# wendongbi/Bridged-GNN

Measured on AMD Instinct MI355X. Metric: aggregated_edges_per_sec_ktgnn_fwd, higher is better.
Workload: dtype f32; 1 GPU; C4 synthetic bridged graph (local) N=1000000 E'=20991058, 2-layer KT-GNN eval fwd F=128 hidden=128 C=2; parallelism=single, execution=eager launches

## Files before the change

bridged_gnn_amd/_lib.py:

```python
import ctypes as C
import os

import torch

_HERE = os.path.dirname(os.path.abspath(__file__))
SO_PATH = os.path.join(_HERE, "csrc", "libbgnn_hip.so")
_lib = None

_P, _I64, _I32, _F32, _SZ, _INT = C.c_void_p, C.c_int64, C.c_int32, C.c_float, C.c_size_t, C.c_int

SIGNATURES = {
    "bgnn_version": (_INT, []),
    "bgnn_source_hash": (C.c_char_p, []),
    "bgnn_error_string": (C.c_char_p, [_INT]),
    "bgnn_csr_workspace_bytes": (_SZ, [_I64, _I64]),
    "bgnn_build_dst_csr": (_INT, [_P, _I64, _I64, _INT, _P, _P, _P, _P, _P, _SZ, _P]),
    "bgnn_domain_sums_f64": (_INT, [_P, _I64, _I32, _I64, _P, _P, _P]),
    "bgnn_domain_sums_workspace_bytes": (_SZ, [_I32]),
    "bgnn_domain_sums_ws_f64": (_INT, [_P, _I64, _I32, _I64, _P, _P, _P, _SZ, _P]),
    "bgnn_domain_delta_f32": (_INT, [_P, _I32, _P, _P]),
    "bgnn_adaptedconv_transform_f32": (_INT, [_P, _I64, _I32, _I64, _P, _P, _I32, _I32, _P, _P, _P, _P,
                                               _P, _P, _P, _P, _I64, _I64, _P, _P]),
    "bgnn_adaptedconv_transform_sums_f32": (_INT, [_P, _I64, _I32, _I64, _P, _P, _I32, _I32, _P, _P, _P, _P,
                                                    _P, _P, _P, _P, _I64, _I64, _I64, _I64, _P, _P]),
# ... 4 lines not shown
    "bgnn_classifier_stage_f32": (_INT, [_P, _I64, _I32, _I64, _P, _P, _I32, _I32, _P, _P, _P, _P, _P, _P, _P, _P, _I64, _I64,
                                          _P, _P, _I32, _INT, _P, _P, _P, _P, _P, _P]),
    "bgnn_linear_narrow_transform_f32": (_INT, [_P, _I64, _I32, _I64, _P, _P, _I32, _INT, _P, _P, _P, _P, _P, _P]),
    "bgnn_narrow_transform_finish_f32": (_INT, [_P, _I64, _P, _P, _I32, _P, _P, _P, _P, _P, _P, _I64, _P, _P]),
    "bgnn_gram_workspace_bytes": (C.c_size_t, [_I32, _I32]),
    "bgnn_gram_f32": (_INT, [_P, _I64, _I32, _P, _I64, _I32, _I64, _P, _P, C.c_size_t, _P]),
    "bgnn_transform_bwd_prep_workspace_bytes": (C.c_size_t, [_I64, _I32]),
    "bgnn_transform_bwd_prep_f32": (_INT, [_P, _I64, _I64, _I32, _P, _P, _I64, _I32, _P, _P, _P, _P, _P, _P, _I32, _I64, _P, _I64, _P, _P, C.c_size_t, _P]),
    "bgnn_bn_acc_doubles": (_I64, [_I32]),
    "bgnn_bn_relu_dropout_f32": (_INT, [_P, _I64, _I32, _I64, _P, _P, _F32, _INT, _F32, C.c_uint64, _P, _F32, _P, _P, _P, _I64, _P, _P]),
    "bgnn_bn_relu_dropout_bwd_f32": (_INT, [_P, _P, _I64, _I32, _I64, _I64, _P, _P, _P, _F32, _INT, _F32, C.c_uint64, _P, _P, _I64, _P, _P]),
    "bgnn_bn_colstats_f32": (_INT, [_P, _I64, _I32, _I64, _P, _P]),
    "bgnn_bn_apply_rows_f32": (_INT, [_P, _I64, _I32, _I64, _P, _I64, _P, _P, _F32, _INT, _F32, C.c_uint64, _P, _P, _I64, _F32, _P, _P, _P, _I64, _P]),
    "bgnn_bn_bwd_reduce_rows_f32": (_INT, [_P, _P, _I64, _I32, _I64, _I64, _P, _I64, _P, _P, _F32, _INT, _F32, C.c_uint64, _P, _P, _I64, _P, _P]),
    "bgnn_bn_bwd_apply_rows_f32": (_INT, [_P, _P, _I64, _I32, _I64, _I64, _P, _P, _I64, _P, _P, _F32, _INT, _F32, C.c_uint64, _P, _P, _I64, _P, _I64, _P]),
    "bgnn_transform_bwd_consts_f32": (_INT, [_P, _P, _P, _P, _P, _I32, _I32, _P, _P, _P, _P]),
    "bgnn_transform_bwd_finish_f32": (_INT, [_P, _P, _P, _P, _P, _P, _P, _I32, _I32, _I32, _P, _P, _P, _P, _P, _P, _P, _I64, _P]),
    "bgnn_rowdot_f32": (_INT, [_P, _I64, _I64, _I32, _P, _I64, _I32, _P, _P]),
    "bgnn_linear_f32": (_INT, [_P, _I64, _I32, _I64, _P, _P, _I32, _INT, _P, _P, _P, _I64, _P]),
    "bgnn_adaptedconv_aggregate_f32": (_INT, [_P, _P, _I64, _P, _P, _P, _P, _P, _I64, _I64, _I32, _F32,
                                               _P, _I64, _P, _P, _P, _INT, _P, _INT, _I64, _I32, _P, _P, _P]),
    "bgnn_adaptedconv_aggregate_bounded_f32": (_INT, [_P, _P, _I64, _P, _P, _P, _P, _P, _I64, _I64, _I32, _F32,
                                                       _P, _I64, _P, _P, _P, _INT, _P, _INT, _I64, _I32, _P, _P, _I64, _I32, _P]),
    "bgnn_aggregate_hub_workspace_bytes": (C.c_size_t, [_I64, _I32, _I64]),
    "bgnn_adaptedconv_aggregate_hub_f32": (_INT, [_P, _P, _I64, _P, _P, _P, _P, _P, _I64, _I32, _F32, _P, _I64, _P, _P, _INT, _P, _I32, _P,
                                                   _P, _I32, _P, _I64, _P, _P, _P, _I64, _P, _P, C.c_size_t, _P]),
    "bgnn_adaptedconv_aggregate_bwd_f32": (_INT, [_P, _P, _I64, _P, _P, _P, _P, _P, _I64, _I64, _I32, _F32,
                                                   _P, _I64, _P, _P, _I64, _P, _P, _P, _P, _P]),
    "bgnn_aggregate_bwd_pull_workspace_bytes": (C.c_size_t, [_I64, _I64, _I64, _I32, _I64, _I64]),
    "bgnn_adaptedconv_aggregate_bwd_pull_f32": (_INT, [_P, _P, _I64, _P, _P, _P, _P, _P, _P, _P, _P, _I64, _I64, _I32, _F32,
                                                        _P, _I64, _P, _P, _I64, _P, _P, _P, _P, _I32,
                                                        _P, _I64, _P, _P, _P, _I64, _P, _I64, _P, _P, _P, _I64, _P, C.c_size_t, _P]),
    "bgnn_aggregate_heads_bwd_workspace_bytes": (C.c_size_t, [_I64, _I64, _I32, _I64, _I64]),
    "bgnn_adaptedconv_aggregate_heads_bwd_f32": (_INT, [_P, _P, _P, _P, _P, _P, _P, _P, _P, _I64, _I64, _I32, _I32, _F32,
                                                         _P, _P, _P, _INT, _P, _P, _P, _P, _I32,
                                                         _P, _I64, _P, _P, _P, _I64, _P, _I64, _P, _P, _P, _I64, _P, C.c_size_t, _P]),
    "bgnn_adaptedconv_aggregate_heads_wide_f32": (_INT, [_P, _P, _I64, _P, _P, _P, _P, _P, _I64, _I32, _I32, _F32, _P, _P, _P]),
    "bgnn_aggregate_heads_wide_bwd_workspace_bytes": (C.c_size_t, [_I64, _I32, _I64]),
    "bgnn_adaptedconv_aggregate_heads_wide_bwd_f32": (_INT, [_P, _P, _I64, _P, _P, _P, _P, _P, _P, _P, _I64, _I32, _I32, _F32,
                                                              _P, _P, _P, _P, _P, _P, _P, _P, C.c_size_t, _P]),
    "bgnn_l2_normalize_rows_f32": (_INT, [_P, _I64, _I32, _F32, _P, _P]),
    "bgnn_topk_workspace_bytes": (_SZ, [_I64, _I64, _I32]),
    "bgnn_cosine_topk_f32": (_INT, [_P, _P, _I64, _I64, _I32, _I32, _INT, _P, _P, _P, _P, _SZ, _P]),
    "bgnn_mlp_pair_topk_f32": (_INT, [_P, _P, _P, _P, _P, _F32, _I64, _I64, _I32, _I32, _INT, _P, _P, _P,
                                       _P, _SZ, _P]),
    "bgnn_topk_edges_i64": (_INT, [_P, _I64, _I32, _I64, _I64, _P, _P]),
# ... 175 lines not shown
```

bridged_gnn_amd/csrc/bgnn_aggregate.hip:

```cpp
#include <cstdlib>
#include "bgnn_common.h"

namespace {

struct AggParams {
  const float* h_t2s;
  const float* h_s2t;
  int64_t ldh;
  const float* a_t2s;
  const float* a_s2t;
  const int32_t* rowptr;
  const int32_t* col;
  const uint8_t* mask;
  int64_t row_begin;
  int64_t row_end;
  int32_t D;
  float slope;
  float* out;
  int64_t ldo;
  float* alpha;
  const float* ep_scale;
  const float* ep_shift;
  int ep_relu;
  unsigned int* tile_queue;
  double* colsum;
  int32_t heads;
  float* state_ms;
  int mode;
  int64_t park_begin;
  int tq_chunk;
  int tq_interleave;
  int xcd_segments;
  const int32_t* vrow_node;
  const int32_t* vrow_bounds;
  int64_t n_vrows;
  float* vout; float* vms;
  int32_t hub_threshold;
  const char* tbl_base;
  uint32_t tbl_bytes, off_t2s, off_s2t;
  int32_t gather_hint;
  uint32_t dead_off;
};

__device__ __forceinline__ float leaky(float v, float slope) { return v > 0.f ? v : v * slope; }

template <int LF, int EP, int U>
__global__ __launch_bounds__(256) void agg_kernel(AggParams p) {
  constexpr int GL = LF * EP;
  constexpr int GPW = 64 / GL;
  constexpr int RPB = 4 * GPW;
  const int lane = threadIdx.x & 63;
  const int wave = threadIdx.x >> 6;
  const int g = lane / GL;
  const int lg = lane % GL;
  const int sub = lg / LF;
  const int f0 = (lg % LF) * 4;
  const bool fvalid = f0 < p.D;

  const int64_t ntiles = ((p.row_end - p.row_begin) * p.heads + RPB - 1) / RPB;
  bgnn::XcdRange tr = bgnn::xcd_pos_range(ntiles);
  __shared__ float red[2][LF * 4 + 1];
  if (p.colsum != nullptr) {
    for (int t = threadIdx.x; t < 2 * (LF * 4 + 1); t += 256) (&red[0][0])[t] = 0.f;
    __syncthreads();
// ... 429 lines not shown
      if (p.colsum != nullptr) {
        if (dom_s) { cs_s.x += o.x; cs_s.y += o.y; cs_s.z += o.z; cs_s.w += o.w; n_s += 1.f; }
        else       { cs_t.x += o.x; cs_t.y += o.y; cs_t.z += o.z; cs_t.w += o.w; n_t += 1.f; }
      }
    }
  }
  if (p.colsum != nullptr) {
    unsafeAtomicAdd(&red[0][f0], cs_s.x); unsafeAtomicAdd(&red[0][f0 + 1], cs_s.y);
    unsafeAtomicAdd(&red[0][f0 + 2], cs_s.z); unsafeAtomicAdd(&red[0][f0 + 3], cs_s.w);
    unsafeAtomicAdd(&red[1][f0], cs_t.x); unsafeAtomicAdd(&red[1][f0 + 1], cs_t.y);
    unsafeAtomicAdd(&red[1][f0 + 2], cs_t.z); unsafeAtomicAdd(&red[1][f0 + 3], cs_t.w);
    if (lg == 0) { unsafeAtomicAdd(&red[0][LF * 4], n_s); unsafeAtomicAdd(&red[1][LF * 4], n_t); }
    __syncthreads();
    for (int t = threadIdx.x; t < 2 * (LF * 4 + 1); t += 256) {
      const int d = t / (LF * 4 + 1), c = t % (LF * 4 + 1);
      const double sum = (double)red[d][c];
      if (c == LF * 4) unsafeAtomicAdd(&p.colsum[2 * p.ldo + d], sum);
      else if (c < p.ldo) unsafeAtomicAdd(&p.colsum[d * p.ldo + c], sum);
    }
  }
}

typedef unsigned int u32x4_t __attribute__((ext_vector_type(4)));

template <int CTRL>
__device__ __forceinline__ uint32_t dpp_movu(uint32_t x) { return (uint32_t)__builtin_amdgcn_update_dpp(0, (int)x, CTRL, 0xF, 0xF, true); }

template <int LF, bool ALPHA>
__global__ __launch_bounds__(256) void agg_wide_fast_kernel(AggParams p) {
  static_assert(LF == 16 || LF == 32 || LF == 64, "wide rows only");
  constexpr int U = 4;
  constexpr int GPW = 64 / LF;
  constexpr int RPB = 4 * GPW;
  const int lane = threadIdx.x & 63;
  const int wave = threadIdx.x >> 6;
  const int g = lane / LF;
  const int lg = lane % LF;
  const int f0 = lg * 4;
  const bool fvalid = f0 < p.D;
  const int f0c = fvalid ? f0 : 0;
  const int k = lane & (U - 1);
  const bool b0 = lane & 1, b1 = lane & 2;

  const int32_t row0 = (int32_t)p.row_begin, row1 = (int32_t)p.row_end;
  const int32_t ntiles = (row1 - row0 + RPB - 1) / RPB;
  __shared__ float red[2][LF * 4 + 1];
  if (p.colsum != nullptr) {
    for (int t = threadIdx.x; t < 2 * (LF * 4 + 1); t += 256) (&red[0][0])[t] = 0.f;
    __syncthreads();
  }
  __shared__ unsigned int dyn_tile;
  const uint32_t nstride = (uint32_t)(p.ldh * 4);
  const uint32_t ostride = (uint32_t)(p.ldo * 4);
  const __amdgpu_buffer_rsrc_t rt = __builtin_amdgcn_make_buffer_rsrc(const_cast<char*>(p.tbl_base), (short)0, (int)p.tbl_bytes, 0x00020000);
  const __amdgpu_buffer_rsrc_t ro = __builtin_amdgcn_make_buffer_rsrc(p.out, (short)0, (int)((uint32_t)row1 * ostride), 0x00020000);
  const f2 sl = {p.slope, p.slope};
  float sc4[4] = {0.f, 0.f, 0.f, 0.f}, sh4[4] = {0.f, 0.f, 0.f, 0.f};
  if (p.ep_scale != nullptr) {
#pragma unroll
    for (int c = 0; c < 4; ++c)
      if (f0 + c < p.D) { sc4[c] = p.ep_scale[f0 + c]; sh4[c] = p.ep_shift[f0 + c]; }
  }
  f2 cs_s01 = {0.f, 0.f}, cs_s23 = cs_s01, cs_t01 = cs_s01, cs_t23 = cs_s01;
  float n_s = 0.f, n_t = 0.f;
  f2 aS01 = {0.f, 0.f}, aS23 = aS01, aT01 = aS01, aT23 = aS01;
  if (fvalid) {
    aS01.x = p.a_t2s[f0]; aS01.y = f0 + 1 < p.D ? p.a_t2s[f0 + 1] : 0.f;
    aS23.x = f0 + 2 < p.D ? p.a_t2s[f0 + 2] : 0.f; aS23.y = f0 + 3 < p.D ? p.a_t2s[f0 + 3] : 0.f;
    aT01.x = p.a_s2t[f0]; aT01.y = f0 + 1 < p.D ? p.a_s2t[f0 + 1] : 0.f;
    aT23.x = f0 + 2 < p.D ? p.a_s2t[f0 + 2] : 0.f; aT23.y = f0 + 3 < p.D ? p.a_s2t[f0 + 3] : 0.f;
  }
  const int32_t TQ_CHUNK = p.tq_chunk;
  const int32_t xcd = blockIdx.x % 8, slot = blockIdx.x / 8;
  const int32_t G = ((int32_t)gridDim.x + 7 - xcd) / 8;
  const int32_t tstride = p.tq_interleave ? G : 1;
  const int32_t NSEG = p.xcd_segments > 1 ? p.xcd_segments : 1;
  const int32_t per_x = (ntiles + 7) / 8, seg_len = (per_x + NSEG - 1) / NSEG;
  const int32_t xbase = xcd * per_x;
  const int32_t xend = NSEG > 1 ? xbase + NSEG * seg_len : min((xcd + 1) * per_x, ntiles);
  int32_t tile = xbase + slot - G;
  int32_t chunk_left = 0;
  for (;;) {
    if (p.tile_queue != nullptr) {
      if (chunk_left == 0) {
        __syncthreads();
        if (threadIdx.x == 0) dyn_tile = atomicAdd(&p.tile_queue[xcd], 1u);
        __syncthreads();
        const uint32_t kq = dyn_tile;
        if (p.tq_interleave) {
          const int32_t sc = (int32_t)kq / G, r = (int32_t)kq - sc * G;
          tile = xbase + sc * (TQ_CHUNK * G) + r;
        } else {
          tile = xbase + (int32_t)kq * TQ_CHUNK;
        }
        chunk_left = TQ_CHUNK;
        if (tile >= xend) break;
      } else {
        tile += tstride;
      }
      --chunk_left;
      if (tile >= xend) { chunk_left = 0; continue; }
    } else {
      tile += G;
      if (tile >= xend) break;
    }
    int32_t gt = tile;
    if (NSEG > 1) {
      const int32_t j = tile - xbase, sg = j / seg_len;
      gt = (sg * 8 + xcd) * seg_len + (j - sg * seg_len);
      if (gt >= ntiles) continue;
    }
    const int32_t i0 = row0 + gt * RPB + wave * GPW + g;
    const bool rvalid = i0 < row1;
    const int32_t ic = rvalid ? i0 : row0;
    const bool dom_s = p.mask[ic] != 0;
    const int32_t beg = rvalid ? p.rowptr[ic] : 0;
    const int32_t end = rvalid ? p.rowptr[ic + 1] : 0;
    const uint32_t lbase = (dom_s ? p.off_t2s : p.off_s2t) + (uint32_t)f0c * 4u;
    const f2 a01 = dom_s ? aS01 : aT01, a23 = dom_s ? aS23 : aT23;
    const float4 hi4 = __builtin_bit_cast(float4, __builtin_amdgcn_raw_buffer_load_b128(rt, lbase + __umul24((uint32_t)ic, nstride), 0, 0));
    f2 h01 = {hi4.x, hi4.y}, h23 = {hi4.z, hi4.w};

    float m = -INFINITY, s = 0.f;
    f2 acc01 = {0.f, 0.f}, acc23 = {0.f, 0.f};
    const int32_t niter = (end - beg + U - 1) / U;
    auto issue = [&](float4 (&v)[U], uint32_t off) {
      v[0] = __builtin_bit_cast(float4, __builtin_amdgcn_raw_buffer_load_b128(rt, lbase + dpp_movu<0x00>(off), 0, 0));
      v[1] = __builtin_bit_cast(float4, __builtin_amdgcn_raw_buffer_load_b128(rt, lbase + dpp_movu<0x55>(off), 0, 0));
      v[2] = __builtin_bit_cast(float4, __builtin_amdgcn_raw_buffer_load_b128(rt, lbase + dpp_movu<0xAA>(off), 0, 0));
      v[3] = __builtin_bit_cast(float4, __builtin_amdgcn_raw_buffer_load_b128(rt, lbase + dpp_movu<0xFF>(off), 0, 0));
      asm volatile("" : "+v"(h01), "+v"(h23) : : "memory");
      __builtin_amdgcn_sched_barrier(0);
    };
// ... 42 lines not shown
#define BGNN_ACC(u, w)                                               \
      {                                                              \
        acc01.x = fmaf(w, v[u].x, acc01.x); acc01.y = fmaf(w, v[u].y, acc01.y); \
        acc23.x = fmaf(w, v[u].z, acc23.x); acc23.y = fmaf(w, v[u].w, acc23.y); \
      }
#ifdef AGGF_X_NOACC
      acc01.x += pe * v[0].x + v[1].y + v[2].z + v[3].w;
#else
      { const float w = quad_bcast<0>(pe); BGNN_ACC(0, w) }
      { const float w = quad_bcast<1>(pe); BGNN_ACC(1, w) }
      { const float w = quad_bcast<2>(pe); BGNN_ACC(2, w) }
      { const float w = quad_bcast<3>(pe); BGNN_ACC(3, w) }
#endif
#undef BGNN_ACC
      m = mn;
    };
    int32_t nw = __builtin_amdgcn_readlane(niter, 0);
    if constexpr (LF <= 32) nw = max(nw, __builtin_amdgcn_readlane(niter, 32));
    if constexpr (LF <= 16) nw = max(nw, max(__builtin_amdgcn_readlane(niter, 16), __builtin_amdgcn_readlane(niter, 48)));
    int32_t e = beg + k;
    bool ok = e < end;
    uint32_t myoff = p.dead_off;
    if (nw > 0) myoff = row_off((uint32_t)p.col[max(min(e, end - 1), 0)], ok);
    for (int32_t it = 0; it < nw; ++it) {
      float4 v[U];
      issue(v, myoff);
      const int32_t e_cur = e;
      e += U;
      const bool ok2 = e < end;
      uint32_t nextid = load_id(e);
      update(v, ok, e_cur);
      ok = ok2;
      take_id(nextid);
      myoff = row_off(nextid, ok);
    }
    s += bgnn::dpp_mov<0xB1>(s);
    s += bgnn::dpp_mov<0x4E>(s);

    const float inv = 1.f / (s + 1e-16f);
    if constexpr (ALPHA) {
      if (lg < U) {
        for (int32_t e2 = beg + lg; e2 < end; e2 += 4 * U) {
          float a[4];
#pragma unroll
          for (int j = 0; j < 4; ++j) a[j] = e2 + j * U < end ? p.alpha[e2 + j * U] : 0.f;
#pragma unroll
          for (int j = 0; j < 4; ++j)
            if (e2 + j * U < end) p.alpha[e2 + j * U] = __expf(a[j] - m) * inv;
        }
      }
    }
    if (rvalid && f0 < p.ldo) {
      float4 o = make_float4(acc01.x * inv, acc01.y * inv, acc23.x * inv, acc23.y * inv);
      if (p.ep_scale != nullptr) {
        o.x = fmaf(o.x, sc4[0], sh4[0]); o.y = fmaf(o.y, sc4[1], sh4[1]);
        o.z = fmaf(o.z, sc4[2], sh4[2]); o.w = fmaf(o.w, sc4[3], sh4[3]);
      }
// ... 231 lines not shown
  return 0;
}

static bool fast_plan(AggParams& p, int64_t table_rows) {
  static const bool on = [] { const char* e = getenv("BGNN_AGG_FAST"); return !(e && atoi(e) == 0); }();
  if (!on || table_rows <= 0) return false;
  if (p.heads != 1 || p.mode != 0 || p.n_vrows != 0 || p.hub_threshold != 0) return false;
  const int64_t lim24 = (int64_t)1 << 24, lim32 = ((int64_t)1 << 32) - 1;
  if (table_rows > lim24 || p.row_end > table_rows || p.ldh * 4 >= lim24 || p.ldo * 4 >= lim24) return false;
  const char* a = reinterpret_cast<const char*>(p.h_t2s);
  const char* b = reinterpret_cast<const char*>(p.h_s2t);
  const char* lo = a < b ? a : b;
  const int64_t span = (int64_t)((a < b ? b : a) - lo) + table_rows * p.ldh * 4;
  if (span > lim32 || p.row_end * p.ldo * 4 > lim32) return false;
  p.tbl_base = lo;
  p.tbl_bytes = (uint32_t)span;
  p.off_t2s = (uint32_t)(a - lo);
  p.off_s2t = (uint32_t)(b - lo);
  const int64_t lane_max = (span - table_rows * p.ldh * 4) + p.ldh * 4, dead = (((int64_t)1 << 32) - 16) - lane_max;
  p.dead_off = dead >= span ? (uint32_t)dead : 0u;
  return true;
}

template <int LF, bool ALPHA>
int launch_wide_fast(const AggParams& p, hipStream_t st) {
  constexpr int RPB = 4 * (64 / LF);
  static const int per_cu_max = [] {
    int per_cu = 0;
    if (hipOccupancyMaxActiveBlocksPerMultiprocessor(&per_cu, agg_wide_fast_kernel<LF, ALPHA>, 256, 0) != hipSuccess || per_cu < 1) return 0;
    if (per_cu > 8) per_cu = 8;
    const char* e = getenv("BGNN_AGG_BLOCKS_PER_CU");
    if (e && atoi(e) > 0 && atoi(e) < per_cu) per_cu = atoi(e);
    return per_cu;
  }();
  static const int n_cu = [] {
    int dev = 0;
    hipDeviceProp_t prop;
    if (hipGetDevice(&dev) != hipSuccess || hipGetDeviceProperties(&prop, dev) != hipSuccess) return 0;
    return prop.multiProcessorCount;
  }();
  static const bool forced = getenv("BGNN_AGG_BLOCKS_PER_CU") != nullptr;
  int per_cu = per_cu_max;
  if (p.gather_hint == 2 && !forced && per_cu > 3) per_cu = 3;
  const int64_t cap = (per_cu_max > 0 && n_cu > 0) ? (int64_t)per_cu * n_cu / 8 * 8 : 2048;
  const int64_t ntiles = (p.row_end - p.row_begin + RPB - 1) / RPB;
  int64_t grid = ntiles < cap ? (ntiles + 7) / 8 * 8 : cap;
  if (grid < 8) grid = 8;
  AggParams q = p;
  q.tq_chunk = tq_chunk_for(ntiles, grid);
  static const int il = [] { const char* e = getenv("BGNN_AGG_INTERLEAVE"); return e ? atoi(e) : 1; }();
  q.tq_interleave = il;
  static const int nseg = [] { const char* e = getenv("BGNN_XCD_SEGMENTS"); return e ? atoi(e) : 8; }();
  q.xcd_segments = nseg;
  hipLaunchKernelGGL((agg_wide_fast_kernel<LF, ALPHA>), dim3((unsigned)grid), dim3(256), 0, st, q);
  BGNN_LAUNCH_CHECK();
  return 0;
}

struct HubMergeParams {
  const int32_t* hub_rows; const int32_t* seg_ptr; int64_t n_hubs;
  const float* part_acc;
  const float* part_ms;
  const uint8_t* mask;
  int32_t D; int64_t ldo; int32_t heads;
  float* out; const float* ep_scale; const float* ep_shift; int ep_relu;
  double* colsum; float* state_ms;
  float* alpha; const int32_t* rowptr;
};

template <int LF>
__global__ __launch_bounds__(256) void hub_merge_wide_kernel(HubMergeParams p) {
  const int lane = threadIdx.x % LF, grp = threadIdx.x / LF;
  constexpr int GPB = 256 / LF;
  const int f0 = lane * 4;
  const bool fvalid = f0 < p.D;
  __shared__ float red[2][LF * 4 + 1];
// ... 137 lines not shown
    if (nv <= 32) return launch_wide<32, 4>(p, st);
    return launch_wide<64, 4>(p, st);
  }
  if (nv <= 16) return launch<16, 1, 8>(p, st);
  if (nv <= 32) return launch<32, 1, 4>(p, st);
  return launch<64, 1, 4>(p, st);
}

static bool hub_capable(int32_t D, int64_t ldh, int64_t ldo, int32_t heads, float slope) {
  if ((heads == 3 || heads == 2) && D <= 4 && ldh == 4 && ldo == 4) return true;
  const int nv = (D + 3) / 4;
  return heads == 1 && nv > 8 && slope >= 0.f && slope <= 1.f && ldh * 4 < (int64_t)1 << 32;
}

}

static int aggregate_impl(const float* h_t2s, const float* h_s2t, int64_t ldh,
                          const float* a_t2s, const float* a_s2t,
                          const int32_t* rowptr, const int32_t* col, const uint8_t* mask,
                          int64_t row_begin, int64_t row_end, int32_t D, float negative_slope,
                          float* out, int64_t ldo, float* alpha_opt,
                          const float* ep_scale_opt, const float* ep_shift_opt, int ep_relu,
                          float* state_ms_opt, int part, int64_t park_begin, int32_t heads,
                          double* colsum_opt, uint32_t* tile_queue_opt, int64_t table_rows, int32_t gather_hint, void* stream) {
  if (colsum_opt && heads != 1) return BGNN_E_SHAPE;
  if (part == 1 && (park_begin < row_begin || park_begin > row_end)) return BGNN_E_SHAPE;
  if (part < 0 || part > 3 || (part != 0 && (!state_ms_opt || alpha_opt))) return BGNN_E_NULL;
  if (part == 3 && !((heads == 3 || heads == 2) && D <= 4 && ldh == 4 && ldo == 4)) return BGNN_E_SHAPE;
  if (heads < 1 || heads > 8 || (heads > 1 && (alpha_opt || ep_scale_opt))) return BGNN_E_SHAPE;
  if (ep_relu < 0 || ep_relu > 2) return BGNN_E_SHAPE;
  if (ep_relu == 2 && !((heads == 3 || heads == 2) && D <= 4 && ldh == 4 && ldo == 4)) return BGNN_E_SHAPE;
  if (!h_t2s || !h_s2t || !a_t2s || !a_s2t || !rowptr || !col || !mask || !out) return BGNN_E_NULL;
  if (row_begin < 0 || row_end < row_begin || D <= 0 || D > 256 || ldh < D || ldo < D) return BGNN_E_SHAPE;
  if ((ldh & 3) || (ldo & 3) || !bgnn_aligned16(h_t2s) || !bgnn_aligned16(h_s2t) || !bgnn_aligned16(out))
    return BGNN_E_ALIGN;
  if ((ep_scale_opt == nullptr) != (ep_shift_opt == nullptr)) return BGNN_E_NULL;
  if (row_end == row_begin) return 0;
  AggParams p{h_t2s, h_s2t, ldh, a_t2s, a_s2t, rowptr, col, mask, row_begin, row_end, D, negative_slope,
              out, ldo, alpha_opt, ep_scale_opt, ep_shift_opt, ep_relu, tile_queue_opt, colsum_opt, heads, state_ms_opt, part,
              park_begin, 4};
  p.gather_hint = gather_hint;
  hipStream_t st = (hipStream_t)stream;
  if (tile_queue_opt) {
    hipError_t e = bgnn_zero_async(tile_queue_opt, 8 * sizeof(uint32_t), st);
    if (e != hipSuccess) return (int)e;
  }
  return dispatch_aggregate(p, st, table_rows);
}

extern "C" int bgnn_adaptedconv_aggregate_f32(const float* h_t2s, const float* h_s2t, int64_t ldh,
                                              const float* a_t2s, const float* a_s2t,
                                              const int32_t* rowptr, const int32_t* col, const uint8_t* mask,
                                              int64_t row_begin, int64_t row_end, int32_t D, float negative_slope,
                                              float* out, int64_t ldo, float* alpha_opt,
                                              const float* ep_scale_opt, const float* ep_shift_opt, int ep_relu,
                                              float* state_ms_opt, int part, int64_t park_begin, int32_t heads,
                                              double* colsum_opt, uint32_t* tile_queue_opt, void* stream) {
  return aggregate_impl(h_t2s, h_s2t, ldh, a_t2s, a_s2t, rowptr, col, mask, row_begin, row_end, D, negative_slope, out, ldo, alpha_opt,
                        ep_scale_opt, ep_shift_opt, ep_relu, state_ms_opt, part, park_begin, heads, colsum_opt, tile_queue_opt, 0, 0, stream);
}

extern "C" int bgnn_adaptedconv_aggregate_bounded_f32(const float* h_t2s, const float* h_s2t, int64_t ldh,
                                                      const float* a_t2s, const float* a_s2t,
                                                      const int32_t* rowptr, const int32_t* col, const uint8_t* mask,
                                                      int64_t row_begin, int64_t row_end, int32_t D, float negative_slope,
                                                      float* out, int64_t ldo, float* alpha_opt,
                                                      const float* ep_scale_opt, const float* ep_shift_opt, int ep_relu,
                                                      float* state_ms_opt, int part, int64_t park_begin, int32_t heads,
                                                      double* colsum_opt, uint32_t* tile_queue_opt, int64_t table_rows, int32_t gather_hint,
                                                      void* stream) {
  if (table_rows < row_end || gather_hint < 0 || gather_hint > 2) return BGNN_E_SHAPE;
  return aggregate_impl(h_t2s, h_s2t, ldh, a_t2s, a_s2t, rowptr, col, mask, row_begin, row_end, D, negative_slope, out, ldo, alpha_opt,
                        ep_scale_opt, ep_shift_opt, ep_relu, state_ms_opt, part, park_begin, heads, colsum_opt, tile_queue_opt, table_rows, gather_hint, stream);
}

extern "C" size_t bgnn_aggregate_hub_workspace_bytes(int64_t n_segments, int32_t heads, int64_t ldo) {
  const size_t nv = (size_t)(n_segments > 0 ? n_segments : 0), h = (size_t)(heads > 0 ? heads : 1);
  return bgnn_align_up(sizeof(float) * nv * h * (size_t)(ldo > 0 ? ldo : 0), 256) + bgnn_align_up(sizeof(float) * 2 * nv * h, 256) + 256;
}

extern "C" int bgnn_adaptedconv_aggregate_hub_f32(const float* h_t2s, const float* h_s2t, int64_t ldh,
                                                  const float* a_t2s, const float* a_s2t,
                                                  const int32_t* rowptr, const int32_t* col, const uint8_t* mask,
                                                  int64_t N, int32_t D, float negative_slope, float* out, int64_t ldo,
                                                  const float* ep_scale_opt, const float* ep_shift_opt, int ep_relu,
                                                  float* state_ms_opt, int32_t heads, double* colsum_opt,
                                                  uint32_t* tile_queue_opt, int32_t hub_threshold, const int32_t* hub_rows,
                                                  int64_t n_hubs, const int32_t* hub_seg_ptr, const int32_t* seg_bounds,
                                                  const int32_t* seg_node, int64_t n_segments, float* alpha_opt,
                                                  void* ws, size_t ws_bytes, void* stream) {
  if (!h_t2s || !h_s2t || !a_t2s || !a_s2t || !rowptr || !col || !mask || !out) return BGNN_E_NULL;
  if (alpha_opt && heads != 1) return BGNN_E_SHAPE;
  if (n_hubs > 0 && (!hub_rows || !hub_seg_ptr || !seg_bounds || !seg_node || !ws)) return BGNN_E_NULL;
  if (N < 0 || D <= 0 || D > 256 || ldh < D || ldo < D || (ldh & 3) || (ldo & 3) || hub_threshold < 2 || n_hubs < 0 || n_segments < n_hubs)
    return BGNN_E_SHAPE;
  if (!hub_capable(D, ldh, ldo, heads, negative_slope)) return BGNN_E_SHAPE;
// ... 84 lines not shown
```

bridged_gnn_amd/ops.py:

```python
import ctypes
import os

import torch

from . import _lib as L

__all__ = ["DstCSR", "build_dst_csr", "domain_delta", "pack_transform_heads", "adaptedconv_transform", "adaptedconv_aggregate", "linear", "linear_supported", "linear_narrow_supported", "linear_narrow_transform", "narrow_transform_finish", "gram", "gram_supported", "rowdot", "transform_bwd_prep", "topk_edges_coalesced",
           "l2_normalize_rows", "cosine_topk", "mlp_pair_topk", "topk_edges", "coalesce", "gather_rows", "pad4",
           "sage_mean_aggregate", "sage_mean_aggregate_bwd", "rows_segment_add", "gcn_aggregate", "gcn_aggregate_bwd", "gat_scores", "gat_aggregate", "gat_aggregate_bwd", "gatv2_aggregate", "gatv2_aggregate_bwd", "wide_heads_supported",
           "adaptedconv_aggregate_heads_wide", "adaptedconv_aggregate_heads_wide_bwd", "pair_csr", "pair_mlp_stats", "pair_mlp_loss",
           "pair_mlp_segsum", "pair_mlp_eval", "pair_mlp_count", "PAIR_MLP_WIDTH", "pair_cos_loss", "pair_cos_segsum", "pair_cos_count",
           "PAIR_COS_WIDTH"]


def pad4(n):
    return (int(n) + 3) // 4 * 4


HUB_THRESHOLD = 128
HUB_SEGMENT = 64


class DstCSR:

# ... 512 lines not shown
    if tile_need is not None:
        if delta is not None or tuple(tail_single) != (0, 0):
            raise ValueError("tile_need needs the sums form of the transform and no tail_single")
        if tile_need.dtype != torch.int32 or tile_need.numel() != (N + 31) // 32:
            raise ValueError("tile_need: one int32 per 32-row tile")
        fn, name, tail = lib.bgnn_adaptedconv_transform_need_f32, "bgnn_adaptedconv_transform_need_f32", (L.ptr(tile_need),)
    if delta is None and H == 1 and (tile_need is not None or tail_single[0] or tail_single[1]):
        c = getattr(tile_need, "_team_plan", None)
        runs = c[1] if (c is not None and c[0] == (N, dev, tile_need._version)) else transform_team_runs(N, dev, tile_need, tail_single)
        if runs:
            flat = (ctypes.c_int64 * (3 * len(runs)))(*[v for r in runs for v in r])
            fn, name = lib.bgnn_adaptedconv_transform_need2_f32, "bgnn_adaptedconv_transform_need2_f32"
            tail = (int(tail_single[0]), int(tail_single[1]), L.ptr(tile_need) if tile_need is not None else None, flat, len(runs))
    rc = fn(L.ptr(x), N, Din, x.stride(0), L.ptr(mask_u8), L.ptr(first), H, D, L.ptr(Wp), L.ptr(bp), L.ptr(gates), L.ptr(gconst),
            L.ptr_rows(out[0][1]), L.ptr_rows(out[0][0]), L.ptr_rows(o1[1]), L.ptr_rows(o1[0]), ldh, row_stride, *tail,
            L.ptr(small), L.stream())
    L.check(rc, name)
    return out


_P2_STATIC = os.environ.get("BGNN_P2_STATIC", "1") != "0"


def _tile_queue(dev):
    return torch.empty(8, dtype=torch.int32, device=dev)


def heads_log_softmax_supported(heads, D):
    return heads in (2, 3) and D <= 4


def _hub_shape_ok(D, ldh, ldo, heads, slope):
    if heads in (2, 3) and D <= 4 and ldh == 4 and ldo == 4:
        return True
    return heads == 1 and D > 32 and 0.0 <= slope <= 1.0


def adaptedconv_aggregate(h_t2s, h_s2t, a_t2s, a_s2t, csr, mask_u8, D, negative_slope=0.1, n_dst=None,
                          want_alpha=False, ep_scale=None, ep_shift=None, ep_relu=False, out=None,
                          row_begin=0, row_end=None, state_ms=None, part=0, heads=1, colsum=None, log_softmax=False,
                          park_begin=None):
    lib = L.lib()
    n_dst = csr.num_nodes if n_dst is None else int(n_dst)
    row_end = n_dst if row_end is None else int(row_end)
    ldh = h_t2s.stride(0) // heads
    ldo = pad4(D)
    dev = h_t2s.device
    if out is None:
# ... 1 lines not shown
    assert h_t2s.stride(0) == h_s2t.stride(0) and h_t2s.stride(0) % heads == 0 and out.stride(0) % heads == 0
    alpha = torch.empty(csr.num_edges, dtype=torch.float32, device=dev) if want_alpha else None
    tq = _tile_queue(dev) if heads == 1 else None
    if row_end <= int(row_begin):
        return (out, alpha) if want_alpha else out
    if ((not want_alpha or heads == 1) and part in (0, 3) and int(row_begin) == 0 and row_end == csr.num_nodes == n_dst and h_t2s.shape[0] == n_dst
            and (ep_scale is None or heads == 1) and _hub_shape_ok(D, ldh, out.stride(0) // heads, heads, negative_slope)
            and os.environ.get("BGNN_HUB_ROWS", "1") != "0"):
        hubs = csr.hub_tables()
        if hubs is not None:
            hub_rows, seg_ptr, seg_bounds, seg_node = hubs
            nseg = int(seg_node.numel())
            wsb = lib.bgnn_aggregate_hub_workspace_bytes(nseg, heads, out.stride(0) // heads)
            ws = torch.empty(wsb, dtype=torch.uint8, device=dev)
            rc = lib.bgnn_adaptedconv_aggregate_hub_f32(
                L.ptr_rows(h_t2s), L.ptr_rows(h_s2t), ldh, L.ptr(a_t2s), L.ptr(a_s2t), L.ptr(csr.rowptr), L.ptr(csr.col),
                L.ptr(mask_u8), n_dst, D, float(negative_slope), L.ptr_rows(out), out.stride(0) // heads,
                L.ptr(ep_scale), L.ptr(ep_shift), 2 if log_softmax else (1 if ep_relu else 0),
                L.ptr(state_ms) if part == 3 else None, int(heads), L.ptr(colsum),
                L.ptr(tq), HUB_THRESHOLD, L.ptr(hub_rows), int(hub_rows.numel()),
                L.ptr(seg_ptr), L.ptr(seg_bounds), L.ptr(seg_node), nseg, L.ptr(alpha), L.ptr(ws), wsb, L.stream())
            L.check(rc, "bgnn_adaptedconv_aggregate_hub_f32")
            return (out, alpha) if want_alpha else out
    rc = lib.bgnn_adaptedconv_aggregate_bounded_f32(
        L.ptr_rows(h_t2s), L.ptr_rows(h_s2t), ldh, L.ptr(a_t2s), L.ptr(a_s2t), L.ptr(csr.rowptr), L.ptr(csr.col),
        L.ptr(mask_u8), int(row_begin), row_end, D, float(negative_slope), L.ptr_rows(out), out.stride(0) // heads, L.ptr(alpha),
        L.ptr(ep_scale), L.ptr(ep_shift), 2 if log_softmax else (1 if ep_relu else 0), L.ptr(state_ms), int(part),
        int(row_begin) if park_begin is None else int(park_begin), int(heads), L.ptr(colsum),
        L.ptr(tq) if not (part == 2 and _P2_STATIC) else None, min(int(h_t2s.shape[0]), int(h_s2t.shape[0])),
        csr.gather_hint() if (heads == 1 and D > 32 and part == 0) else 0, L.stream())
    L.check(rc, "bgnn_adaptedconv_aggregate_bounded_f32")
    return (out, alpha) if want_alpha else out


def _bwd_hub_args(csr, use=True):
    use = use and os.environ.get("BGNN_HUB_ROWS", "1") != "0"
    args, nseg = [HUB_THRESHOLD], []
    for tables in ((csr.hub_tables(), csr.transposed_hub_tables()) if use else (None, None)):
        rows, seg_ptr, bounds, node = tables if tables is not None else (None, None, None, None)
        nseg.append(0 if tables is None else int(node.numel()))
        args += [L.ptr(rows), 0 if tables is None else int(rows.numel()), L.ptr(seg_ptr), L.ptr(bounds), L.ptr(node), nseg[-1]]
    return args, nseg[0], nseg[1]


def adaptedconv_aggregate_bwd(h_t2s, h_s2t, a_t2s, a_s2t, csr, mask_u8, D, out, alpha, grad_out, negative_slope=0.1):
    lib = L.lib()
    dev = h_t2s.device
    da_t2s = torch.zeros(D, dtype=torch.float32, device=dev)
    da_s2t = torch.zeros(D, dtype=torch.float32, device=dev)
    grad_out = grad_out.contiguous()
    ldh, ldo, ldg = h_t2s.stride(0), out.stride(0), grad_out.stride(0)
    pull = D <= 256 and ldg % 4 == 0 and grad_out.data_ptr() % 16 == 0 and h_t2s.shape[0] == csr.num_nodes
    if pull and D > 128:
        pull = (ldh % 4 == 0 and ldo % 4 == 0 and h_t2s.data_ptr() % 16 == 0 and h_s2t.data_ptr() % 16 == 0
# ... 859 lines not shown
```

include/bgnn.h:

```cpp
#ifndef BGNN_H_
#define BGNN_H_
#include <stddef.h>
#include <stdint.h>

#ifdef __cplusplus
extern "C" {
#endif

#define BGNN_VERSION 114
#define BGNN_E_NULL (-1)
#define BGNN_E_SHAPE (-2)
#define BGNN_E_WORKSPACE (-3)
#define BGNN_E_ALIGN (-4)
#define BGNN_E_RANGE (-5)

int bgnn_version(void);
const char* bgnn_error_string(int code);
const char* bgnn_source_hash(void);

size_t bgnn_csr_workspace_bytes(int64_t N, int64_t E);
int bgnn_build_dst_csr(const int64_t* edge_index, int64_t E, int64_t N, int rewrite_self_loops,
                       int32_t* rowptr, int32_t* col, int32_t* eperm_opt, int64_t* E_out_dev,
                       void* ws, size_t ws_bytes, void* stream);

// ... 88 lines not shown
                                         float* h_s2t_0, float* h_t2s_0, float* h_s2t_1, float* h_t2s_1,
                                         int64_t ldh, int64_t row_stride, int64_t n_tail_t2s, int64_t n_tail_s2t,
                                         const int32_t* tile_need_opt, const int64_t* team_runs_host_opt, int32_t n_team_runs,
                                         float* small_ws, void* stream);

int bgnn_adaptedconv_aggregate_f32(const float* h_t2s, const float* h_s2t, int64_t ldh,
                                   const float* a_t2s, const float* a_s2t,
                                   const int32_t* rowptr, const int32_t* col, const uint8_t* mask,
                                   int64_t row_begin, int64_t row_end, int32_t D, float negative_slope,
                                   float* out, int64_t ldo, float* alpha_opt,
                                   const float* ep_scale_opt, const float* ep_shift_opt, int ep_relu,
                                   float* state_ms_opt, int part, int64_t park_begin, int32_t heads, double* colsum_opt,
                                   uint32_t* tile_queue_opt, void* stream);

int bgnn_adaptedconv_aggregate_bounded_f32(const float* h_t2s, const float* h_s2t, int64_t ldh,
                                           const float* a_t2s, const float* a_s2t,
                                           const int32_t* rowptr, const int32_t* col, const uint8_t* mask,
                                           int64_t row_begin, int64_t row_end, int32_t D, float negative_slope,
                                           float* out, int64_t ldo, float* alpha_opt,
                                           const float* ep_scale_opt, const float* ep_shift_opt, int ep_relu,
                                           float* state_ms_opt, int part, int64_t park_begin, int32_t heads, double* colsum_opt,
                                           uint32_t* tile_queue_opt, int64_t table_rows, int32_t gather_hint, void* stream);

size_t bgnn_aggregate_hub_workspace_bytes(int64_t n_segments, int32_t heads, int64_t ldo);
int bgnn_adaptedconv_aggregate_hub_f32(const float* h_t2s, const float* h_s2t, int64_t ldh,
                                       const float* a_t2s, const float* a_s2t,
                                       const int32_t* rowptr, const int32_t* col, const uint8_t* mask,
                                       int64_t N, int32_t D, float negative_slope, float* out, int64_t ldo,
                                       const float* ep_scale_opt, const float* ep_shift_opt, int ep_relu,
                                       float* state_ms_opt, int32_t heads, double* colsum_opt,
                                       uint32_t* tile_queue_opt, int32_t hub_threshold, const int32_t* hub_rows,
                                       int64_t n_hubs, const int32_t* hub_seg_ptr, const int32_t* seg_bounds,
                                       const int32_t* seg_node, int64_t n_segments, float* alpha_opt,
                                       void* ws, size_t ws_bytes, void* stream);

int bgnn_adaptedconv_aggregate_bwd_f32(const float* h_t2s, const float* h_s2t, int64_t ldh,
                                       const float* a_t2s, const float* a_s2t,
                                       const int32_t* rowptr, const int32_t* col, const uint8_t* mask,
                                       int64_t row_begin, int64_t row_end, int32_t D, float negative_slope,
                                       const float* out, int64_t ldo, const float* alpha,
                                       const float* grad_out, int64_t ldg,
                                       float* dh_t2s, float* dh_s2t, float* da_t2s, float* da_s2t,
                                       void* stream);

size_t bgnn_aggregate_bwd_pull_workspace_bytes(int64_t N, int64_t E, int64_t ldh, int32_t D, int64_t d_segments, int64_t s_segments);
int bgnn_adaptedconv_aggregate_bwd_pull_f32(const float* h_t2s, const float* h_s2t, int64_t ldh,
// ... 210 lines not shown
```

Baseline: 51.55 billion edges/s.

## Replace chunked tile queue with per-wave prefetched tile claims over sharded subqueues

The wide aggregation kernel now claims work one tile at a time from several padded per-XCD subqueue counters instead of claiming chunks behind a block-wide __syncthreads. Waves take turns issuing the atomic for a future tile, overlap it with their gather loop, and publish the result through a small LDS ring read by the other waves. The intent is to remove block-level barriers and chunk-granularity load imbalance on the power-law edge distribution. The cost is extra atomics per tile, spin-waits on LDS, and inline-asm exec manipulation that could stall or race if the ring handshake is wrong.

```diff
diff --git a/bridged_gnn_amd/_lib.py b/bridged_gnn_amd/_lib.py
--- a/bridged_gnn_amd/_lib.py
+++ b/bridged_gnn_amd/_lib.py
@@ -50,6 +50,9 @@
                                                _P, _I64, _P, _P, _P, _INT, _P, _INT, _I64, _I32, _P, _P, _P]),
     "bgnn_adaptedconv_aggregate_bounded_f32": (_INT, [_P, _P, _I64, _P, _P, _P, _P, _P, _I64, _I64, _I32, _F32,
                                                        _P, _I64, _P, _P, _P, _INT, _P, _INT, _I64, _I32, _P, _P, _I64, _I32, _P]),
+    "bgnn_aggregate_tile_queue_words": (_I64, []),
+    "bgnn_adaptedconv_aggregate_queued_f32": (_INT, [_P, _P, _I64, _P, _P, _P, _P, _P, _I64, _I64, _I32, _F32,
+                                                      _P, _I64, _P, _P, _P, _INT, _P, _INT, _I64, _I32, _P, _P, _I64, _I64, _I32, _P]),
     "bgnn_aggregate_hub_workspace_bytes": (C.c_size_t, [_I64, _I32, _I64]),
     "bgnn_adaptedconv_aggregate_hub_f32": (_INT, [_P, _P, _I64, _P, _P, _P, _P, _P, _I64, _I32, _F32, _P, _I64, _P, _P, _INT, _P, _I32, _P,
                                                    _P, _I32, _P, _I64, _P, _P, _P, _I64, _P, _P, C.c_size_t, _P]),
diff --git a/bridged_gnn_amd/csrc/bgnn_aggregate.hip b/bridged_gnn_amd/csrc/bgnn_aggregate.hip
--- a/bridged_gnn_amd/csrc/bgnn_aggregate.hip
+++ b/bridged_gnn_amd/csrc/bgnn_aggregate.hip
@@ -1,4 +1,5 @@
 #include <cstdlib>
+#include <cstring>
 #include "bgnn_common.h"
 
 namespace {
@@ -40,6 +41,9 @@
   uint32_t tbl_bytes, off_t2s, off_s2t;
   int32_t gather_hint;
   uint32_t dead_off;
+  int64_t tq_words;
+  int tq_subqueues;
+  int tq_ahead;
 };
 
 __device__ __forceinline__ float leaky(float v, float slope) { return v > 0.f ? v : v * slope; }
@@ -515,6 +519,7 @@
 }
 
 typedef unsigned int u32x4_t __attribute__((ext_vector_type(4)));
+constexpr int TQ_SPACING_WORDS = 32;
 
 template <int CTRL>
 __device__ __forceinline__ uint32_t dpp_movu(uint32_t x) { return (uint32_t)__builtin_amdgcn_update_dpp(0, (int)x, CTRL, 0xF, 0xF, true); }
@@ -538,10 +543,13 @@
   const int32_t row0 = (int32_t)p.row_begin, row1 = (int32_t)p.row_end;
   const int32_t ntiles = (row1 - row0 + RPB - 1) / RPB;
   __shared__ float red[2][LF * 4 + 1];
-  if (p.colsum != nullptr) {
+  __shared__ unsigned long long cl_ring[4];
+  __shared__ uint32_t cl_prog[4];
+  const bool tile_claims = p.tile_queue != nullptr && p.tq_subqueues > 0;
+  if (tile_claims && threadIdx.x < 4) { cl_ring[threadIdx.x] = 0ull; cl_prog[threadIdx.x] = 0u; }
+  if (p.colsum != nullptr)
     for (int t = threadIdx.x; t < 2 * (LF * 4 + 1); t += 256) (&red[0][0])[t] = 0.f;
-    __syncthreads();
-  }
+  if (p.colsum != nullptr || tile_claims) __syncthreads();
   __shared__ unsigned int dyn_tile;
   const uint32_t nstride = (uint32_t)(p.ldh * 4);
   const uint32_t ostride = (uint32_t)(p.ldo * 4);
@@ -573,8 +581,62 @@
   const int32_t xend = NSEG > 1 ? xbase + NSEG * seg_len : min((xcd + 1) * per_x, ntiles);
   int32_t tile = xbase + slot - G;
   int32_t chunk_left = 0;
+  const int32_t NQ = tile_claims ? min((int32_t)p.tq_subqueues, G) : 0;
+  const int32_t wave_u = __builtin_amdgcn_readfirstlane(wave);
+  uint32_t* const qctr = NQ > 0 ? p.tile_queue + (xcd * NQ + slot % NQ) * TQ_SPACING_WORDS : nullptr;
+  const int32_t qpos0 = xbase + (NQ > 0 ? slot % NQ : 0);
+  uint32_t cl_n = 0;
+  uint32_t cl_val = 0;
+  bool cl_own = false, cl_pending = false;
+  bool cl_ending = false, cl_stop = false;
+  auto cl_issue = [&](uint32_t& v) {
+    uint64_t ex;
+    asm volatile("s_mov_b64 %1, exec\n\ts_mov_b64 exec, 1\n\tglobal_atomic_add %0, %2, %3, %4 sc0\n\ts_mov_b64 exec, %1"
+                 : "+v"(v), "=&s"(ex) : "v"(0u), "v"(1u), "s"(qctr) : "memory");
+  };
+  auto cl_wait = [&](uint32_t& v) { asm volatile("s_waitcnt vmcnt(0)" : "+v"(v) : : "memory"); };
+  auto cl_publish = [&](uint32_t tn, uint32_t v) {
+    while (tn >= 4u) {
+      const uint32_t mn = min(min(__hip_atomic_load(&cl_prog[0], __ATOMIC_RELAXED, __HIP_MEMORY_SCOPE_WORKGROUP),
+                                  __hip_atomic_load(&cl_prog[1], __ATOMIC_RELAXED, __HIP_MEMORY_SCOPE_WORKGROUP)),
+                              min(__hip_atomic_load(&cl_prog[2], __ATOMIC_RELAXED, __HIP_MEMORY_SCOPE_WORKGROUP),
+                                  __hip_atomic_load(&cl_prog[3], __ATOMIC_RELAXED, __HIP_MEMORY_SCOPE_WORKGROUP)));
+      if ((uint32_t)__builtin_amdgcn_readfirstlane(mn) + 3u >= tn) break;
+      __builtin_amdgcn_s_sleep(1);
+    }
+    __builtin_amdgcn_fence(__ATOMIC_RELEASE, "workgroup", "local");
+    if (lane == 0)
+      __hip_atomic_store(&cl_ring[tn & 3u], ((unsigned long long)(tn + 1u) << 32) | v, __ATOMIC_RELAXED, __HIP_MEMORY_SCOPE_WORKGROUP);
+  };
+  if (NQ > 0 && wave_u < 2) {
+    uint32_t v = 0;
+    cl_issue(v);
+    cl_wait(v);
+    cl_publish((uint32_t)wave_u, v);
+  }
   for (;;) {
-    if (p.tile_queue != nullptr) {
+    if (NQ > 0) {
+      if (cl_stop) break;
+      uint32_t tag, kq;
+      for (;;) {
+        const unsigned long long w = __hip_atomic_load(&cl_ring[cl_n & 3u], __ATOMIC_RELAXED, __HIP_MEMORY_SCOPE_WORKGROUP);
+        tag = (uint32_t)__builtin_amdgcn_readfirstlane((uint32_t)(w >> 32));
+        kq = (uint32_t)__builtin_amdgcn_readfirstlane((uint32_t)w);
+        if (tag == cl_n + 1u) break;
+        __builtin_amdgcn_s_sleep(1);
+      }
+      __builtin_amdgcn_fence(__ATOMIC_ACQUIRE, "workgroup", "local");
+      if (lane == 0) __hip_atomic_store(&cl_prog[wave], cl_n + 1u, __ATOMIC_RELAXED, __HIP_MEMORY_SCOPE_WORKGROUP);
+      tile = qpos0 + (int32_t)kq * NQ;
+      cl_stop = cl_ending;
+      cl_own = !cl_ending && ((cl_n + 2u) & 3u) == (uint32_t)wave_u;
+      ++cl_n;
+      if (tile >= xend) {
+        if (cl_stop) break;
+        cl_ending = true;
+        continue;
+      }
+    } else if (p.tile_queue != nullptr) {
       if (chunk_left == 0) {
         __syncthreads();
         if (threadIdx.x == 0) dyn_tile = atomicAdd(&p.tile_queue[xcd], 1u);
@@ -601,7 +663,15 @@
     if (NSEG > 1) {
       const int32_t j = tile - xbase, sg = j / seg_len;
       gt = (sg * 8 + xcd) * seg_len + (j - sg * seg_len);
-      if (gt >= ntiles) continue;
+      if (gt >= ntiles) {
+        if (cl_own) {
+          uint32_t v = 0;
+          cl_issue(v);
+          cl_wait(v);
+          cl_publish(cl_n + 1u, v);
+        }
+        continue;
+      }
     }
     const int32_t i0 = row0 + gt * RPB + wave * GPW + g;
     const bool rvalid = i0 < row1;
@@ -690,6 +760,12 @@
     bool ok = e < end;
     uint32_t myoff = p.dead_off;
     if (nw > 0) myoff = row_off((uint32_t)p.col[max(min(e, end - 1), 0)], ok);
+    asm volatile("" : "+v"(h01), "+v"(h23) : : "memory");
+    if (cl_own) {
+      cl_issue(cl_val);
+      if (p.tq_ahead) cl_pending = true;
+      else { cl_wait(cl_val); cl_publish(cl_n + 1u, cl_val); }
+    }
     for (int32_t it = 0; it < nw; ++it) {
       float4 v[U];
       issue(v, myoff);
@@ -700,7 +776,18 @@
       update(v, ok, e_cur);
       ok = ok2;
       take_id(nextid);
+      if (cl_pending) {
+        asm volatile("" : "+v"(cl_val) : : "memory");
+        cl_publish(cl_n + 1u, cl_val);
+        cl_pending = false;
+        __builtin_amdgcn_sched_barrier(0);
+      }
       myoff = row_off(nextid, ok);
+    }
+    if (cl_pending) {
+      cl_wait(cl_val);
+      cl_publish(cl_n + 1u, cl_val);
+      cl_pending = false;
     }
     s += bgnn::dpp_mov<0xB1>(s);
     s += bgnn::dpp_mov<0x4E>(s);
@@ -978,6 +1065,20 @@
   return true;
 }
 
+constexpr int kClaimTileDefault = 1;
+struct ClaimCfg { int tile, nq, ahead; };
+static const ClaimCfg& claim_cfg() {
+  static const ClaimCfg c = [] {
+    ClaimCfg r{kClaimTileDefault, 4, 1};
+    if (const char* e = getenv("BGNN_AGG_CLAIM")) r.tile = strcmp(e, "chunk") == 0 ? 0 : (strcmp(e, "tile") == 0 ? 1 : r.tile);
+    if (const char* e = getenv("BGNN_AGG_SUBQUEUES")) { const int v = atoi(e); if (v >= 1 && v <= 8) r.nq = v; }
+    if (const char* e = getenv("BGNN_AGG_CLAIM_AHEAD")) r.ahead = atoi(e) != 0;
+    return r;
+  }();
+  return c;
+}
+static int64_t claim_queue_words() { return (int64_t)8 * claim_cfg().nq * TQ_SPACING_WORDS; }
+
 template <int LF, bool ALPHA>
 int launch_wide_fast(const AggParams& p, hipStream_t st) {
   constexpr int RPB = 4 * (64 / LF);
@@ -1008,6 +1109,10 @@
   q.tq_interleave = il;
   static const int nseg = [] { const char* e = getenv("BGNN_XCD_SEGMENTS"); return e ? atoi(e) : 8; }();
   q.xcd_segments = nseg;
+  const ClaimCfg& cc = claim_cfg();
+  const bool tile_claims = cc.tile && p.tile_queue != nullptr && p.tq_words >= claim_queue_words();
+  q.tq_subqueues = tile_claims ? cc.nq : 0;
+  q.tq_ahead = cc.ahead;
   hipLaunchKernelGGL((agg_wide_fast_kernel<LF, ALPHA>), dim3((unsigned)grid), dim3(256), 0, st, q);
   BGNN_LAUNCH_CHECK();
   return 0;
@@ -1191,8 +1296,10 @@
                           float* out, int64_t ldo, float* alpha_opt,
                           const float* ep_scale_opt, const float* ep_shift_opt, int ep_relu,
                           float* state_ms_opt, int part, int64_t park_begin, int32_t heads,
-                          double* colsum_opt, uint32_t* tile_queue_opt, int64_t table_rows, int32_t gather_hint, void* stream) {
+                          double* colsum_opt, uint32_t* tile_queue_opt, int64_t tile_queue_words, int64_t table_rows, int32_t gather_hint,
+                          void* stream) {
   if (colsum_opt && heads != 1) return BGNN_E_SHAPE;
+  if (tile_queue_opt && tile_queue_words < 8) return BGNN_E_WORKSPACE;
   if (part == 1 && (park_begin < row_begin || park_begin > row_end)) return BGNN_E_SHAPE;
   if (part < 0 || part > 3 || (part != 0 && (!state_ms_opt || alpha_opt))) return BGNN_E_NULL;
   if (part == 3 && !((heads == 3 || heads == 2) && D <= 4 && ldh == 4 && ldo == 4)) return BGNN_E_SHAPE;
@@ -1209,9 +1316,11 @@
               out, ldo, alpha_opt, ep_scale_opt, ep_shift_opt, ep_relu, tile_queue_opt, colsum_opt, heads, state_ms_opt, part,
               park_begin, 4};
   p.gather_hint = gather_hint;
+  p.tq_words = tile_queue_words;
   hipStream_t st = (hipStream_t)stream;
   if (tile_queue_opt) {
-    hipError_t e = bgnn_zero_async(tile_queue_opt, 8 * sizeof(uint32_t), st);
+    const int64_t zw = claim_cfg().tile && tile_queue_words >= claim_queue_words() ? claim_queue_words() : 8;
+    hipError_t e = bgnn_zero_async(tile_queue_opt, (size_t)zw * sizeof(uint32_t), st);
     if (e != hipSuccess) return (int)e;
   }
   return dispatch_aggregate(p, st, table_rows);
@@ -1226,7 +1335,7 @@
                                               float* state_ms_opt, int part, int64_t park_begin, int32_t heads,
                                               double* colsum_opt, uint32_t* tile_queue_opt, void* stream) {
   return aggregate_impl(h_t2s, h_s2t, ldh, a_t2s, a_s2t, rowptr, col, mask, row_begin, row_end, D, negative_slope, out, ldo, alpha_opt,
-                        ep_scale_opt, ep_shift_opt, ep_relu, state_ms_opt, part, park_begin, heads, colsum_opt, tile_queue_opt, 0, 0, stream);
+                        ep_scale_opt, ep_shift_opt, ep_relu, state_ms_opt, part, park_begin, heads, colsum_opt, tile_queue_opt, 8, 0, 0, stream);
 }
 
 extern "C" int bgnn_adaptedconv_aggregate_bounded_f32(const float* h_t2s, const float* h_s2t, int64_t ldh,
@@ -1240,7 +1349,24 @@
                                                       void* stream) {
   if (table_rows < row_end || gather_hint < 0 || gather_hint > 2) return BGNN_E_SHAPE;
   return aggregate_impl(h_t2s, h_s2t, ldh, a_t2s, a_s2t, rowptr, col, mask, row_begin, row_end, D, negative_slope, out, ldo, alpha_opt,
-                        ep_scale_opt, ep_shift_opt, ep_relu, state_ms_opt, part, park_begin, heads, colsum_opt, tile_queue_opt, table_rows, gather_hint, stream);
+                        ep_scale_opt, ep_shift_opt, ep_relu, state_ms_opt, part, park_begin, heads, colsum_opt, tile_queue_opt, 8, table_rows, gather_hint, stream);
+}
+
+extern "C" int64_t bgnn_aggregate_tile_queue_words(void) { return claim_cfg().tile ? claim_queue_words() : 8; }
+
+extern "C" int bgnn_adaptedconv_aggregate_queued_f32(const float* h_t2s, const float* h_s2t, int64_t ldh,
+                                                     const float* a_t2s, const float* a_s2t,
+                                                     const int32_t* rowptr, const int32_t* col, const uint8_t* mask,
+                                                     int64_t row_begin, int64_t row_end, int32_t D, float negative_slope,
+                                                     float* out, int64_t ldo, float* alpha_opt,
+                                                     const float* ep_scale_opt, const float* ep_shift_opt, int ep_relu,
+                                                     float* state_ms_opt, int part, int64_t park_begin, int32_t heads,
+                                                     double* colsum_opt, uint32_t* tile_queue_opt, int64_t tile_queue_words,
+                                                     int64_t table_rows, int32_t gather_hint, void* stream) {
+  if (table_rows < row_end || gather_hint < 0 || gather_hint > 2) return BGNN_E_SHAPE;
+  return aggregate_impl(h_t2s, h_s2t, ldh, a_t2s, a_s2t, rowptr, col, mask, row_begin, row_end, D, negative_slope, out, ldo, alpha_opt,
+                        ep_scale_opt, ep_shift_opt, ep_relu, state_ms_opt, part, park_begin, heads, colsum_opt, tile_queue_opt,
+                        tile_queue_words, table_rows, gather_hint, stream);
 }
 
 extern "C" size_t bgnn_aggregate_hub_workspace_bytes(int64_t n_segments, int32_t heads, int64_t ldo) {
diff --git a/bridged_gnn_amd/ops.py b/bridged_gnn_amd/ops.py
--- a/bridged_gnn_amd/ops.py
+++ b/bridged_gnn_amd/ops.py
@@ -558,8 +558,14 @@
 _P2_STATIC = os.environ.get("BGNN_P2_STATIC", "1") != "0"
 
 
+_TILE_QUEUE_WORDS = None
+
+
 def _tile_queue(dev):
-    return torch.empty(8, dtype=torch.int32, device=dev)
+    global _TILE_QUEUE_WORDS
+    if _TILE_QUEUE_WORDS is None:
+        _TILE_QUEUE_WORDS = max(8, int(L.lib().bgnn_aggregate_tile_queue_words()))
+    return torch.empty(_TILE_QUEUE_WORDS, dtype=torch.int32, device=dev)
 
 
 def heads_log_softmax_supported(heads, D):
@@ -607,14 +613,15 @@
                 L.ptr(seg_ptr), L.ptr(seg_bounds), L.ptr(seg_node), nseg, L.ptr(alpha), L.ptr(ws), wsb, L.stream())
             L.check(rc, "bgnn_adaptedconv_aggregate_hub_f32")
             return (out, alpha) if want_alpha else out
-    rc = lib.bgnn_adaptedconv_aggregate_bounded_f32(
+    queue = tq if not (part == 2 and _P2_STATIC) else None
+    rc = lib.bgnn_adaptedconv_aggregate_queued_f32(
         L.ptr_rows(h_t2s), L.ptr_rows(h_s2t), ldh, L.ptr(a_t2s), L.ptr(a_s2t), L.ptr(csr.rowptr), L.ptr(csr.col),
         L.ptr(mask_u8), int(row_begin), row_end, D, float(negative_slope), L.ptr_rows(out), out.stride(0) // heads, L.ptr(alpha),
         L.ptr(ep_scale), L.ptr(ep_shift), 2 if log_softmax else (1 if ep_relu else 0), L.ptr(state_ms), int(part),
         int(row_begin) if park_begin is None else int(park_begin), int(heads), L.ptr(colsum),
-        L.ptr(tq) if not (part == 2 and _P2_STATIC) else None, min(int(h_t2s.shape[0]), int(h_s2t.shape[0])),
+        L.ptr(queue), 0 if queue is None else int(queue.numel()), min(int(h_t2s.shape[0]), int(h_s2t.shape[0])),
         csr.gather_hint() if (heads == 1 and D > 32 and part == 0) else 0, L.stream())
-    L.check(rc, "bgnn_adaptedconv_aggregate_bounded_f32")
+    L.check(rc, "bgnn_adaptedconv_aggregate_queued_f32")
     return (out, alpha) if want_alpha else out
 
 
diff --git a/include/bgnn.h b/include/bgnn.h
--- a/include/bgnn.h
+++ b/include/bgnn.h
@@ -134,6 +134,17 @@
                                            float* state_ms_opt, int part, int64_t park_begin, int32_t heads, double* colsum_opt,
                                            uint32_t* tile_queue_opt, int64_t table_rows, int32_t gather_hint, void* stream);
 
+int64_t bgnn_aggregate_tile_queue_words(void);
+int bgnn_adaptedconv_aggregate_queued_f32(const float* h_t2s, const float* h_s2t, int64_t ldh,
+                                          const float* a_t2s, const float* a_s2t,
+                                          const int32_t* rowptr, const int32_t* col, const uint8_t* mask,
+                                          int64_t row_begin, int64_t row_end, int32_t D, float negative_slope,
+                                          float* out, int64_t ldo, float* alpha_opt,
+                                          const float* ep_scale_opt, const float* ep_shift_opt, int ep_relu,
+                                          float* state_ms_opt, int part, int64_t park_begin, int32_t heads, double* colsum_opt,
+                                          uint32_t* tile_queue_opt, int64_t tile_queue_words, int64_t table_rows, int32_t gather_hint,
+                                          void* stream);
+
 size_t bgnn_aggregate_hub_workspace_bytes(int64_t n_segments, int32_t heads, int64_t ldo);
 int bgnn_adaptedconv_aggregate_hub_f32(const float* h_t2s, const float* h_s2t, int64_t ldh,
                                        const float* a_t2s, const float* a_s2t,
```

New measurement: 52.52 billion edges/s (median of 6 runs). 1.9% higher.
